# maelaubert/VulkanSift

Hardware: AMD Instinct MI355X
Metric: SIFT detect+match frames/sec (640x480, ~2k kp) (higher is better)
Workload: dtype f32

## Files before the change

### include/vksift_hip.h

```cpp
#ifndef VKSIFT_HIP_H
#define VKSIFT_HIP_H

#include <stddef.h>
#include <stdint.h>

#ifdef __cplusplus
extern "C"
{
#endif

#define VKSIFT_HIP_MAX_TAPS 20
#define VKSIFT_HIP_MATCH_CHUNKS 32
#define VKSIFT_HIP_MATCH_SMALL_NA 1536u
#define VKSIFT_HIP_MATCH_SMALL_NB 4096u
#define VKSIFT_HIP_MATCH_SCRATCH_U32(na, nb) (2u * (size_t)(na) + (size_t)(nb) + 72u + (size_t)(na) * 16u * VKSIFT_HIP_MATCH_CHUNKS)
#define VKSIFT_HIP_ABI_VERSION 6u
#define VKSIFT_HIP_GATHER_SLOTS 512u
#define VKSIFT_HIP_MATCH_SLOTS 256u
#define VKSIFT_HIP_MATCH_PK_NB 32768u
#define VKSIFT_HIP_MAX_ORI 18
#define VKSIFT_HIP_MAX_OCTAVE_SIDE 16383u

  typedef void *vksift_hip_stream;
  typedef void *vksift_hip_graph;
  typedef void *vksift_hip_event;

  int vksift_hip_init(void);
  uint32_t vksift_hip_abi_version(void);
  int vksift_hip_device_count(void);
  int vksift_hip_device_name(int idx, char *out256);
  int vksift_hip_set_device(int idx);
  size_t vksift_hip_device_free_mem(void);
  void *vksift_hip_malloc(size_t bytes);
  void vksift_hip_free(void *p);
  void *vksift_hip_host_malloc(size_t bytes);
  void vksift_hip_host_free(void *p);
  int vksift_hip_host_register(void *p, size_t bytes);
  int vksift_hip_host_unregister(void *p);
  int vksift_hip_is_pinned(const void *p);
  vksift_hip_stream vksift_hip_stream_create(void);
  void vksift_hip_stream_destroy(vksift_hip_stream s);
  int vksift_hip_stream_sync(vksift_hip_stream s);
  int vksift_hip_stream_busy(vksift_hip_stream s);
  vksift_hip_event vksift_hip_event_create(void);
  void vksift_hip_event_destroy(vksift_hip_event e);
  int vksift_hip_event_record(vksift_hip_event e, vksift_hip_stream s);
  int vksift_hip_event_sync(vksift_hip_event e);
  int vksift_hip_event_busy(vksift_hip_event e);
  float vksift_hip_event_elapsed_ms(vksift_hip_event a, vksift_hip_event b);
  int vksift_hip_stream_wait_event(vksift_hip_stream s, vksift_hip_event e);
  int vksift_hip_capture_begin(vksift_hip_stream s);
  int vksift_hip_capture_end(vksift_hip_stream s, vksift_hip_graph *out);
  int vksift_hip_graph_launch(vksift_hip_graph g, vksift_hip_stream s);
  void vksift_hip_graph_destroy(vksift_hip_graph g);
  int vksift_hip_memcpy_h2d(void *dst, const void *src, size_t n, vksift_hip_stream s);
  int vksift_hip_memcpy_d2h(void *dst, const void *src, size_t n, vksift_hip_stream s);
  int vksift_hip_memcpy_d2d(void *dst, const void *src, size_t n, vksift_hip_stream s);
  int vksift_hip_memcpy2d_d2h(void *dst, size_t dpitch, const void *src, size_t spitch, size_t width_bytes, size_t height, vksift_hip_stream s);
  int vksift_hip_post_words(uint32_t *host_mapped_dst, const uint32_t *src, size_t n_words, vksift_hip_stream s);
  int vksift_hip_memset(void *dst, int value, size_t n, vksift_hip_stream s);
  const char *vksift_hip_error_string(int err);
  void vksift_hip_range_push(const char *name);
  void vksift_hip_range_pop(void);

  enum
  {
    VKSIFT_TUNE_WG_TARGET = 0,
    VKSIFT_TUNE_WIDE_MASK = 1,
    VKSIFT_TUNE_MULTI_MAX = 2,
    VKSIFT_TUNE_REFINE_PTR = 3,
    VKSIFT_TUNE_SCAN_FORM = 4,
    VKSIFT_TUNE_PAIR_FORM = 5,
    VKSIFT_TUNE_PYR_GATE = 6,
    VKSIFT_TUNE_DENSE_ROWS = 7,
    VKSIFT_TUNE_SEED_WG = 8,
    VKSIFT_TUNE_SCAN_BAND = 9,
    VKSIFT_TUNE_TAIL_MULTI = 10,
    VKSIFT_TUNE_ZERO_COPY = 11,
    VKSIFT_TUNE_MIN_MARCH = 12,
    VKSIFT_TUNE_COUNT = 16
  };
  int vksift_hip_tune(int knob, int value);
  int vksift_hip_tune_get(int knob);


  typedef struct
  {
    float *base;
    uint32_t w, h;
    uint32_t pitch;
    uint64_t img_stride;
    uint32_t fp16;
    uint32_t reverse;
  } vksift_hip_Plane;

  int vksift_hip_input_blit(const uint8_t *src, uint32_t sw, uint32_t sh, uint64_t src_img_stride, vksift_hip_Plane dst, uint32_t batch,
                            vksift_hip_stream s);

  int vksift_hip_blur(vksift_hip_Plane src, vksift_hip_Plane dst, const float *taps, uint32_t ntaps, uint32_t batch, vksift_hip_stream s);

  int vksift_hip_blur_pair(vksift_hip_Plane src, vksift_hip_Plane dst1, vksift_hip_Plane dst2, const float *taps1, uint32_t ntaps1, const float *taps2,
                           uint32_t ntaps2, uint32_t batch, vksift_hip_stream s);

  int vksift_hip_blur_form(vksift_hip_Plane src, vksift_hip_Plane dst, uint32_t ntaps, uint32_t batch);

  int vksift_hip_blur_multi(const vksift_hip_Plane *src, const vksift_hip_Plane *dst, uint32_t n, const float *taps, uint32_t ntaps, uint32_t batch,
                            vksift_hip_stream s);

  int vksift_hip_blur_downsample(vksift_hip_Plane src, vksift_hip_Plane dst, vksift_hip_Plane next, const float *taps, uint32_t ntaps, uint32_t batch,
                                 vksift_hip_stream s);

  int vksift_hip_seed_upsampled(const uint8_t *src, uint32_t sw, uint32_t sh, uint64_t src_img_stride, vksift_hip_Plane dst, const float *taps, uint32_t ntaps,
                                uint32_t batch, vksift_hip_stream s);

  int vksift_hip_seed_direct(const uint8_t *src, uint32_t sw, uint32_t sh, uint64_t src_img_stride, vksift_hip_Plane dst, const float *taps, uint32_t ntaps,
                             uint32_t batch, vksift_hip_stream s);

  int vksift_hip_downsample(vksift_hip_Plane src, vksift_hip_Plane dst, uint32_t batch, vksift_hip_stream s);

  int vksift_hip_octave_chain(const vksift_hip_Plane *layers, uint32_t n_oct, uint32_t n_layers, uint32_t S, const float *taps, const uint32_t *ntaps,
                              uint32_t batch, vksift_hip_stream s);

  int vksift_hip_dog_plane(const float *lo, const float *hi, uint32_t w, uint32_t h, uint32_t pitch, uint32_t fp16, float *out_dense, vksift_hip_stream s);

  typedef struct
  {
    float *gauss;
    uint32_t fp16;
    uint32_t w, h, pitch;
    uint64_t plane_stride;
    uint64_t img_stride;
    uint32_t S;
    int32_t octave_idx;
    float seed_sigma;
    float dog_threshold;
    float edge_limit;
    uint8_t *feats;
    uint64_t feat_img_stride;
    uint32_t cap;
    uint32_t *found;
    uint32_t found_img_stride;
    uint64_t *seg_mask;
    uint32_t *seg_off;
    uint64_t seg_img_stride;
    uint32_t *cand_xy;
    uint32_t *cand_flag;
    uint32_t *cand_n;
    uint64_t cand_img_stride;
    uint32_t cand_cap;
    float *ori_ang;
    uint32_t *ori_cnt;
    uint64_t ori_img_stride;
    uint32_t max_ori;
    uint32_t use_vlfeat;
    const float *desc_fp_tab;
    uint32_t desc_fp_tab_len;
    uint32_t scan_reverse;
    uint32_t masks_cleared;
    uint32_t sec_index;
  } vksift_hip_OctaveJob;

  typedef struct
  {
    uint8_t *desc;
    uint64_t desc_img_stride;
    uint32_t *norm;
    uint64_t norm_img_stride;
    uint32_t *n;
    uint32_t n_img_stride;
    uint32_t nsec;
    uint32_t sec_cap[16];
    uint8_t *post;
    uint64_t post_img_stride;
    uint32_t *found_post;
    uint32_t found_post_n;
  } vksift_hip_DenseRows;

  int vksift_hip_extract_keypoints(const vksift_hip_OctaveJob *job, uint32_t batch, vksift_hip_stream s, vksift_hip_event scan_done);
  int vksift_hip_orientations(const vksift_hip_OctaveJob *job, uint32_t batch, vksift_hip_stream s);
  int vksift_hip_descriptors(const vksift_hip_OctaveJob *job, uint32_t batch, vksift_hip_stream s);
  int vksift_hip_extract_keypoints_multi(const vksift_hip_OctaveJob *jobs, uint32_t n_jobs, uint32_t batch, vksift_hip_stream s, vksift_hip_event scan_done);
  int vksift_hip_clear_segment_masks(const vksift_hip_OctaveJob *jobs, uint32_t n_jobs, uint32_t batch, vksift_hip_stream s);
  int vksift_hip_selftest_inrange(uint32_t n, uint32_t seed, uint32_t *d_mismatches, vksift_hip_stream s);
  int vksift_hip_orientations_multi(const vksift_hip_OctaveJob *jobs, uint32_t n_jobs, uint32_t batch, vksift_hip_stream s);
  int vksift_hip_descriptors_multi(const vksift_hip_OctaveJob *jobs, uint32_t n_jobs, uint32_t batch, vksift_hip_stream s);
  int vksift_hip_descriptors_multi_dense(const vksift_hip_OctaveJob *jobs, uint32_t n_jobs, uint32_t batch, const vksift_hip_DenseRows *dense,
                                         vksift_hip_stream s);

  int vksift_hip_gather_descriptors(const uint8_t *feats, uint32_t n, uint8_t *desc, vksift_hip_stream s);
  size_t vksift_hip_match_scratch_u32(uint32_t na, uint32_t nb);
  int vksift_hip_match_2nn_desc(const uint8_t *desc_a, uint32_t na, uint32_t a_index_base, const uint8_t *desc_b, uint32_t nb, uint32_t *norm_scratch,
                                size_t scratch_u32, uint8_t *matches, vksift_hip_stream s);
  int vksift_hip_shifted_norms(const uint8_t *desc, uint32_t n, uint32_t *norms, vksift_hip_stream s);
  int vksift_hip_match_2nn_prenormed(const uint8_t *desc_a, const uint32_t *norm_a, uint32_t na, uint32_t a_index_base, const uint8_t *desc_b,
                                     const uint32_t *norm_b, uint32_t nb, uint32_t *scratch, size_t scratch_u32, uint8_t *matches, vksift_hip_stream s);

  int vksift_hip_filter_matches(const uint8_t *fwd, uint64_t fwd_slot_stride, const uint8_t *rev, uint64_t rev_slot_stride, const uint32_t *n_fwd,
                                uint32_t n_stride, float ratio, uint32_t nslots, uint8_t *out, uint64_t out_slot_stride, uint32_t *out_n, vksift_hip_stream s);

  int vksift_hip_pack_features(const uint8_t *feats_base, uint64_t buf_stride, const uint32_t *buf_ids, const uint32_t *out_rows, uint32_t nslots, uint32_t nsec,
                               const uint32_t *sec_off, const uint32_t *sec_cap, const uint32_t *found_base, uint32_t found_buf_stride, uint8_t *out,
                               uint32_t max_rows, uint32_t *found_post, vksift_hip_stream s);
  int vksift_hip_gather_sections(const uint8_t *feats_base, uint64_t buf_stride, const uint32_t *buf_ids, uint32_t nslots, uint32_t nsec,
                                 const uint32_t *sec_off, const uint32_t *sec_cap, const uint32_t *fixed_counts, const uint32_t *found_base,
                                 uint32_t found_buf_stride, uint32_t max_rows, uint32_t pad_rows_to, uint8_t *desc, uint64_t desc_stride,
                                 uint32_t *norms, uint64_t norm_stride, uint32_t *n_out_dev, uint32_t n_stride, vksift_hip_stream s);
  int vksift_hip_match_2nn_async(const uint8_t *cache_desc, const uint32_t *cache_norm, const uint32_t *cache_n, const uint32_t *ids_a, const uint32_t *ids_b,
                                 uint32_t max_na, uint32_t max_nb, uint32_t nb_exact, uint32_t *redo, uint32_t *n_dev, uint8_t *matches, uint32_t nslots, uint64_t cache_desc_stride,
                                 uint64_t cache_norm_stride, uint64_t redo_slot_stride, uint64_t match_slot_stride, uint32_t n_slot_stride,
                                 uint32_t *partial_scratch, vksift_hip_stream s);

  int vksift_hip_gather_correspondences(const uint8_t *feats_base, uint64_t buf_stride, const uint32_t *found_base, uint32_t found_buf_stride,
                                        const uint32_t *slot_tab, const uint32_t *layouts, const uint8_t *filtered, uint64_t filtered_slot_stride,
                                        const uint32_t *filtered_n, uint32_t max_n, uint32_t nslots, float *corr, uint64_t corr_slot_stride, vksift_hip_stream s);
  size_t vksift_hip_ransac_scratch_u32(uint32_t nslots, uint32_t nb_hypotheses);
  int vksift_hip_ransac_homography(const float *corr, uint64_t corr_slot_stride, const uint32_t *n_dev, uint32_t n_stride, uint32_t max_n, uint32_t nslots,
                                   uint32_t nb_hypotheses, float threshold_px, uint64_t seed, uint8_t *results, uint8_t *masks, uint64_t mask_slot_stride,
                                   uint32_t *scratch, size_t scratch_u32, vksift_hip_stream s);
  int vksift_hip_ransac_fundamental(const float *corr, uint64_t corr_slot_stride, const uint32_t *n_dev, uint32_t n_stride, uint32_t max_n, uint32_t nslots,
                                    uint32_t nb_hypotheses, float threshold_px, uint64_t seed, uint8_t *results, uint8_t *masks, uint64_t mask_slot_stride,
                                    uint32_t *scratch, size_t scratch_u32, vksift_hip_stream s);

#define VKSIFT_HIP_GUIDE_HOMOGRAPHY 0u
#define VKSIFT_HIP_GUIDE_FUNDAMENTAL 1u
  int vksift_hip_gather_xy(const uint8_t *feats_base, uint64_t buf_stride, const uint32_t *found_base, uint32_t found_buf_stride, const uint32_t *slot_tab,
                           const uint32_t *layouts, uint32_t max_n, uint32_t nslots, float *xy, uint64_t xy_side_stride, vksift_hip_stream s);
  size_t vksift_hip_guided_scratch_u32(uint32_t nslots, uint32_t max_n);
  int vksift_hip_match_guided(const uint8_t *cache_desc, uint64_t cache_desc_stride, const uint32_t *cache_norm, uint64_t cache_norm_stride, const uint32_t *slot_tab,
                              uint32_t slot_tab_stride, const float *xy, uint64_t xy_side_stride, const uint32_t *n_dev, uint32_t n_stride, uint32_t max_n,
                              const float *models, uint32_t model_stride, const uint32_t *valid, uint32_t valid_stride, uint32_t model_kind, float t2, float ratio,
                              float max_distance, uint32_t cross_check, uint32_t nslots, uint8_t *out, uint64_t out_slot_stride, uint32_t *out_n, uint32_t *scratch,
                              size_t scratch_u32, vksift_hip_stream s);

#ifdef __cplusplus
}
#endif
#endif
```

### vulkansift_amd/csrc/hip/extrema.hip

```cpp
#include <hip/hip_runtime.h>
#include <type_traits>
#include <stdint.h>
#include <stdlib.h>

#include "../detmath.h"
#include "multi.h"
#include "vksift_hip.h"

namespace
{

struct DogView
{
  const float *base;
  int w, h, pitch;
  size_t plane;
  int S;
  int fp16;
};

template <bool F16>
__device__ __forceinline__ float ld(const DogView &d, int s, int x, int y)
{
  if (s < 0 || s > d.S + 1)
    return 0.f;
  if (F16)
  {
    const _Float16 *p = (const _Float16 *)d.base + (size_t)s * d.plane + (size_t)y * d.pitch + x;
    return (float)(_Float16)((float)p[d.plane] - (float)p[0]);
  }
  const float *p = d.base + (size_t)s * d.plane + (size_t)y * d.pitch + x;
  return p[d.plane] - p[0];
}

struct KpRecord
{
  float x, y, scale_x, scale_y;
  uint32_t scale_idx;
  int32_t octave_idx;
  float sigma, orientation, intensity;
};

template <bool F16>
__device__ bool refine_texel(const DogView &d, int x, int y, int s, float dog_threshold, float edge_limit, float seed_sigma, int octave_idx, KpRecord *kp)
{
  const int W = d.w, H = d.h, S = d.S;
  float oX = 0.f, oY = 0.f, oS = 0.f, gX = 0.f, gY = 0.f, gS = 0.f;
  int rx = x, ry = y, rs = s;
  for (int step = 0; step < 5; step++)
  {
    float vc = ld<F16>(d, rs, rx, ry);
    float sp = ld<F16>(d, rs + 1, rx, ry), sm = ld<F16>(d, rs - 1, rx, ry);
    float xp = ld<F16>(d, rs, rx + 1, ry), xm = ld<F16>(d, rs, rx - 1, ry);
    float yp = ld<F16>(d, rs, rx, ry + 1), ym = ld<F16>(d, rs, rx, ry - 1);
    gS = 0.5f * (sp - sm);
    gX = 0.5f * (xp - xm);
    gY = 0.5f * (yp - ym);
    float h11 = sp + sm - 2.f * vc;
    float h22 = xp + xm - 2.f * vc;
    float h33 = yp + ym - 2.f * vc;
    float h12 = 0.25f * (ld<F16>(d, rs + 1, rx + 1, ry) - ld<F16>(d, rs + 1, rx - 1, ry) - ld<F16>(d, rs - 1, rx + 1, ry) + ld<F16>(d, rs - 1, rx - 1, ry));
    float h13 = 0.25f * (ld<F16>(d, rs + 1, rx, ry + 1) - ld<F16>(d, rs + 1, rx, ry - 1) - ld<F16>(d, rs - 1, rx, ry + 1) + ld<F16>(d, rs - 1, rx, ry - 1));
    float h23 = 0.25f * (ld<F16>(d, rs, rx + 1, ry + 1) - ld<F16>(d, rs, rx + 1, ry - 1) - ld<F16>(d, rs, rx - 1, ry + 1) + ld<F16>(d, rs, rx - 1, ry - 1));

    float det = h11 * ((h22 * h33) - (h23 * h23)) - h12 * ((h12 * h33) - (h13 * h23)) + h13 * ((h12 * h23) - (h13 * h22));
    if (det == 0.0f)
      return false;
    float i11 = ((h22 * h33) - (h23 * h23)) / det;
    float i12 = -1.f * ((h12 * h33) - (h13 * h23)) / det;
    float i13 = ((h12 * h23) - (h13 * h22)) / det;
    float i22 = ((h11 * h33) - (h13 * h13)) / det;
    float i23 = -1.f * ((h11 * h23) - (h13 * h12)) / det;
    float i33 = ((h11 * h22) - (h12 * h12)) / det;
    oS = -i11 * gS - i12 * gX - i13 * gY;
    oX = -i12 * gS - i22 * gX - i23 * gY;
    oY = -i13 * gS - i23 * gX - i33 * gY;

    if (fabsf(oX) < 0.6f && fabsf(oY) < 0.6f && fabsf(oS) < 0.6f)
      break;
    else if (step < 4)
    {
      rx += ((oX >= 0.6f && rx < (W - 2)) ? 1 : 0) + ((oX <= -0.6f && rx > 1) ? -1 : 0);
      ry += ((oY >= 0.6f && ry < (H - 2)) ? 1 : 0) + ((oY <= -0.6f && ry > 1) ? -1 : 0);
      rs += ((oS >= 0.6f && rs < (S + 1)) ? 1 : 0) + ((oS <= -0.6f && rs > 1) ? -1 : 0);
    }
  }
  float sx = (float)rx + oX, sy = (float)ry + oY, ss = (float)rs + oS;
  float vc = ld<F16>(d, rs, rx, ry);
  float nv = vc + 0.5f * (gX * oX + gY * oY + gS * oS);
  if (!(fabsf(nv) > dog_threshold && fabsf(oX) < 1.5f && fabsf(oY) < 1.5f && fabsf(oS) < 1.5f && sx >= 0 && sx < (float)W && sy >= 0 && sy < (float)H &&
        ss >= 0 && ss <= (float)(S + 1)))
    return false;
  float e11 = ld<F16>(d, rs, rx + 1, ry) + ld<F16>(d, rs, rx - 1, ry) - 2.f * vc;
  float e22 = ld<F16>(d, rs, rx, ry + 1) + ld<F16>(d, rs, rx, ry - 1) - 2.f * vc;
  float e12 = 0.25f * (ld<F16>(d, rs, rx + 1, ry + 1) - ld<F16>(d, rs, rx + 1, ry - 1) - ld<F16>(d, rs, rx - 1, ry + 1) + ld<F16>(d, rs, rx - 1, ry - 1));
  float edgeness = ((e11 + e22) * (e11 + e22)) / ((e11 * e22) - (e12 * e12));
  if (!((edgeness < edge_limit) && (edgeness >= 0)))
    return false;

  float scale_factor = octave_idx >= 0 ? dm_pow2i(octave_idx) : 1.f / dm_pow2i(-octave_idx);
  kp->scale_x = sx;
  kp->scale_y = sy;
  kp->scale_idx = (uint32_t)roundf(ss);
  kp->octave_idx = octave_idx;
  kp->sigma = seed_sigma * dm_exp2f(ss / (float)S) * scale_factor;
  kp->orientation = 0.f;
  kp->intensity = nv;
  kp->x = sx * scale_factor;
  kp->y = sy * scale_factor;
  return true;
}

template <bool F16>
__device__ bool refine_texel_buf(const __amdgpu_buffer_rsrc_t rsrc, int W, int H, int pitch, unsigned plane, int S, int x, int y, int s, float dog_threshold,
                                 float edge_limit, float seed_sigma, int octave_idx, KpRecord *kp)
{
  constexpr unsigned EB = F16 ? 2u : 4u;
  const int pitch_b = pitch * (int)EB;
  const unsigned plane_b = plane * EB;
  auto tex = [&](unsigned base, int row_off) -> float {
    if (F16)
      return (float)__builtin_bit_cast(_Float16, (unsigned short)__builtin_amdgcn_raw_buffer_load_b16(rsrc, base, row_off, 0));
    return __uint_as_float(__builtin_amdgcn_raw_buffer_load_b32(rsrc, base, row_off, 0));
  };
  auto dog = [&](float hi, float lo) -> float { return F16 ? (float)(_Float16)(hi - lo) : hi - lo; };
  float oX = 0.f, oY = 0.f, oS = 0.f, gX = 0.f, gY = 0.f, gS = 0.f;
  float vc = 0.f, xp = 0.f, xm = 0.f, yp = 0.f, ym = 0.f, h23 = 0.f;
  int rx = x, ry = y, rs = s;
  for (int step = 0; step < 5; step++)
  {
    const unsigned b0 = ((unsigned)rs * plane + (unsigned)(ry - 1) * (unsigned)pitch + (unsigned)(rx - 1)) * EB;
    const unsigned bm = b0 - plane_b, b1 = b0 + plane_b, b2 = b1 + plane_b;
    float g0[3][3], g1[3][3];
#pragma unroll
    for (int j = 0; j < 3; j++)
#pragma unroll
      for (int i = 0; i < 3; i++)
      {
        g0[j][i] = tex(b0 + (unsigned)i * EB, j * pitch_b);
        g1[j][i] = tex(b1 + (unsigned)i * EB, j * pitch_b);
      }
    const float gm_c = tex(bm + EB, pitch_b), gm_xm = tex(bm, pitch_b), gm_xp = tex(bm + 2u * EB, pitch_b), gm_ym = tex(bm + EB, 0), gm_yp = tex(bm + EB, 2 * pitch_b);
    const float g2_c = tex(b2 + EB, pitch_b), g2_xm = tex(b2, pitch_b), g2_xp = tex(b2 + 2u * EB, pitch_b), g2_ym = tex(b2 + EB, 0), g2_yp = tex(b2 + EB, 2 * pitch_b);
    const bool up = rs + 1 <= S + 1;
    const float sp = up ? dog(g2_c, g1[1][1]) : 0.f, sm = dog(g0[1][1], gm_c);
    const float p_xp = up ? dog(g2_xp, g1[1][2]) : 0.f, p_xm = up ? dog(g2_xm, g1[1][0]) : 0.f;
    const float p_yp = up ? dog(g2_yp, g1[2][1]) : 0.f, p_ym = up ? dog(g2_ym, g1[0][1]) : 0.f;
    const float m_xp = dog(g0[1][2], gm_xp), m_xm = dog(g0[1][0], gm_xm), m_yp = dog(g0[2][1], gm_yp), m_ym = dog(g0[0][1], gm_ym);
    float d0[3][3];
#pragma unroll
    for (int j = 0; j < 3; j++)
#pragma unroll
      for (int i = 0; i < 3; i++)
        d0[j][i] = dog(g1[j][i], g0[j][i]);
    vc = d0[1][1];
    xp = d0[1][2], xm = d0[1][0], yp = d0[2][1], ym = d0[0][1];
    gS = 0.5f * (sp - sm);
    gX = 0.5f * (xp - xm);
    gY = 0.5f * (yp - ym);
    float h11 = sp + sm - 2.f * vc;
    float h22 = xp + xm - 2.f * vc;
    float h33 = yp + ym - 2.f * vc;
    float h12 = 0.25f * (p_xp - p_xm - m_xp + m_xm);
    float h13 = 0.25f * (p_yp - p_ym - m_yp + m_ym);
    h23 = 0.25f * (d0[2][2] - d0[0][2] - d0[2][0] + d0[0][0]);

    float det = h11 * ((h22 * h33) - (h23 * h23)) - h12 * ((h12 * h33) - (h13 * h23)) + h13 * ((h12 * h23) - (h13 * h22));
    if (det == 0.0f)
      return false;
    float i11 = ((h22 * h33) - (h23 * h23)) / det;
    float i12 = -1.f * ((h12 * h33) - (h13 * h23)) / det;
    float i13 = ((h12 * h23) - (h13 * h22)) / det;
    float i22 = ((h11 * h33) - (h13 * h13)) / det;
    float i23 = -1.f * ((h11 * h23) - (h13 * h12)) / det;
    float i33 = ((h11 * h22) - (h12 * h12)) / det;
    oS = -i11 * gS - i12 * gX - i13 * gY;
    oX = -i12 * gS - i22 * gX - i23 * gY;
    oY = -i13 * gS - i23 * gX - i33 * gY;

    if (fabsf(oX) < 0.6f && fabsf(oY) < 0.6f && fabsf(oS) < 0.6f)
      break;
    else if (step < 4)
    {
      rx += ((oX >= 0.6f && rx < (W - 2)) ? 1 : 0) + ((oX <= -0.6f && rx > 1) ? -1 : 0);
      ry += ((oY >= 0.6f && ry < (H - 2)) ? 1 : 0) + ((oY <= -0.6f && ry > 1) ? -1 : 0);
      rs += ((oS >= 0.6f && rs < (S + 1)) ? 1 : 0) + ((oS <= -0.6f && rs > 1) ? -1 : 0);
    }
  }
  float sx = (float)rx + oX, sy = (float)ry + oY, ss = (float)rs + oS;
  float nv = vc + 0.5f * (gX * oX + gY * oY + gS * oS);
  if (!(fabsf(nv) > dog_threshold && fabsf(oX) < 1.5f && fabsf(oY) < 1.5f && fabsf(oS) < 1.5f && sx >= 0 && sx < (float)W && sy >= 0 && sy < (float)H &&
        ss >= 0 && ss <= (float)(S + 1)))
    return false;
  float e11 = xp + xm - 2.f * vc;
  float e22 = yp + ym - 2.f * vc;
  float e12 = h23;
  float edgeness = ((e11 + e22) * (e11 + e22)) / ((e11 * e22) - (e12 * e12));
  if (!((edgeness < edge_limit) && (edgeness >= 0)))
    return false;

  float scale_factor = octave_idx >= 0 ? dm_pow2i(octave_idx) : 1.f / dm_pow2i(-octave_idx);
  kp->scale_x = sx;
  kp->scale_y = sy;
  kp->scale_idx = (uint32_t)roundf(ss);
  kp->octave_idx = octave_idx;
  kp->sigma = seed_sigma * dm_exp2f(ss / (float)S) * scale_factor;
  kp->orientation = 0.f;
  kp->intensity = nv;
  kp->x = sx * scale_factor;
  kp->y = sy * scale_factor;
  return true;
}

struct ExtremaArgs
{
  const float *gauss;
  int fp16;
  int w, h, pitch;
  uint64_t plane_stride, img_stride;
  int S, octave_idx;
  float seed_sigma, dog_threshold, edge_limit;
  uint64_t *seg_mask;
  uint32_t *seg_off;
  uint64_t seg_img_stride;
  int nseg;
  uint8_t *feats;
  uint64_t feat_img_stride;
  uint32_t cap;
  uint32_t *found;
  uint32_t found_img_stride;
  uint32_t *cand_xy;
  uint32_t *cand_flag;
  uint32_t *cand_n;
  uint64_t cand_img_stride;
  uint32_t cand_cap;
  int band;
  uint32_t nsegs;
  uint32_t nchunks;
  int scan_rev;
};

__device__ __forceinline__ float wave_shr1(float v, float edge)
{
  return __builtin_bit_cast(float, __builtin_amdgcn_update_dpp(__builtin_bit_cast(int, edge), __builtin_bit_cast(int, v), 0x138, 0xf, 0xf, false));
}
__device__ __forceinline__ float wave_shl1(float v, float edge)
{
  return __builtin_bit_cast(float, __builtin_amdgcn_update_dpp(__builtin_bit_cast(int, edge), __builtin_bit_cast(int, v), 0x130, 0xf, 0xf, false));
}

__device__ __forceinline__ float fmax2(float a, float b)
{
  float r;
  asm("v_max_f32 %0, %1, %2" : "=v"(r) : "v"(a), "v"(b));
  return r;
}
__device__ __forceinline__ float fmin2(float a, float b)
{
  float r;
  asm("v_min_f32 %0, %1, %2" : "=v"(r) : "v"(a), "v"(b));
  return r;
}
__device__ __forceinline__ float fmax3(float a, float b, float c)
{
  float r;
  asm("v_max3_f32 %0, %1, %2, %3" : "=v"(r) : "v"(a), "v"(b), "v"(c));
  return r;
}
__device__ __forceinline__ float fmin3(float a, float b, float c)
{
  float r;
  asm("v_min3_f32 %0, %1, %2, %3" : "=v"(r) : "v"(a), "v"(b), "v"(c));
  return r;
}

__device__ __forceinline__ unsigned long long spread32(unsigned long long x)
{
  x &= 0xFFFFFFFFull;
  x = (x | (x << 16)) & 0x0000FFFF0000FFFFull;
  x = (x | (x << 8)) & 0x00FF00FF00FF00FFull;
  x = (x | (x << 4)) & 0x0F0F0F0F0F0F0F0Full;
  x = (x | (x << 2)) & 0x3333333333333333ull;
  x = (x | (x << 1)) & 0x5555555555555555ull;
  return x;
}

typedef unsigned u32x2_t __attribute__((ext_vector_type(2)));
constexpr unsigned EXT_OOB = 0x80000000u;

template <int S, int NSLOT, bool F16>
__global__ void __launch_bounds__(256, 4) k_extrema_lean(Multi<ExtremaArgs> m, int strip_major)
{
  const VBlock vb = vblock(m);
  const ExtremaArgs &a = m.oct[vb.o];
  const int band = a.band;
  constexpr int NL = S + 2;
  constexpr int EB = F16 ? 2 : 4;
  constexpr int AHEAD = NSLOT - 3;
  const int lane = threadIdx.x & 63;
  const int wv = __builtin_amdgcn_readfirstlane((int)(threadIdx.x >> 6));
  int b = vb.z;
  int bx = vb.x, by = vb.y * 4 + wv;
  if (strip_major)
  {
    unsigned blk = vb.y * vb.gx + vb.x;
    if (strip_major & 2)
    {
      const unsigned per_img = vb.gx * vb.gy, total = per_img * vb.gz;
      if ((total & 7u) == 0)
      {
        const unsigned n = blk + per_img * vb.z, per = total >> 3, k = n >> 3;
        const unsigned wi = (n & 7u) * per + (a.scan_rev ? per - 1u - k : k);
        b = (int)(wi / per_img);
        blk = wi - (unsigned)b * per_img;
      }
    }
    const unsigned id = blk * 4u + (unsigned)wv, ns = (unsigned)(a.nseg + 1) / 2u;
    by = (int)(id / ns), bx = (int)(id - (unsigned)by * ns);
  }
  const int y0 = by * band;
  if (y0 >= a.h)
    return;
  const int y1 = min(y0 + band, a.h);
  const int x0 = bx * 128, x = x0 + 2 * lane;
  const uint8_t *img = (const uint8_t *)a.gauss + (size_t)b * a.img_stride * EB;
  const int pitch4 = a.pitch * EB;
  __amdgpu_buffer_rsrc_t rs[NL + 1];
#pragma unroll
  for (int l = 0; l <= NL; l++)
    rs[l] = __builtin_amdgcn_make_buffer_rsrc((void *)(img + (size_t)l * a.plane_stride * EB), 0, a.pitch * a.h * EB, 0x00020000);
  const unsigned off2 = x < a.pitch ? (unsigned)x * (unsigned)EB : EXT_OOB;
  const int hx = lane == 0 ? x0 - 1 : x0 + 128;
  const unsigned offh = ((lane == 0 || lane == 63) && hx >= 0 && hx < a.pitch) ? (unsigned)hx * (unsigned)EB : EXT_OOB;
  const unsigned long long colA = __ballot(x >= 1 && x < a.w - 1), colB = __ballot(x + 1 < a.w - 1);
  const float pre = a.dog_threshold * 0.8f;
  const int seg0 = bx * 2;
  const bool has_seg1 = seg0 + 1 < a.nseg;
  const int ylo = max(y0, 1), yhi = min(y1, a.h - 1);
  const bool odd = lane & 1;
  const unsigned half = (unsigned)lane >> 1;

  u32x2_t wv2[NSLOT][NL + 1];
  unsigned wh[NSLOT][NL + 1];
  auto fetch_row = [&](int r, auto SLOT) {
    constexpr int slot = decltype(SLOT)::value;
    const int rr = min(max(r, 0), a.h - 1);
    const int so = rr * pitch4;
#pragma unroll
    for (int l = 0; l <= NL; l++)
    {
      if (F16)
      {
        wv2[slot][l].x = __builtin_amdgcn_raw_buffer_load_b32(rs[l], off2, so, 0);
        wh[slot][l] = (unsigned)__builtin_amdgcn_raw_buffer_load_b16(rs[l], offh, so, 0);
      }
      else
      {
        wv2[slot][l] = __builtin_amdgcn_raw_buffer_load_b64(rs[l], off2, so, 0);
        wh[slot][l] = __builtin_amdgcn_raw_buffer_load_b32(rs[l], offh, so, 0);
      }
    }
  };
  typedef _Float16 h2x __attribute__((ext_vector_type(2)));
  auto to_dog = [&](auto SLOT) {
    constexpr int slot = decltype(SLOT)::value;
    if (F16)
    {
      float lo0, lo1, loh;
      {
        const h2x t = __builtin_bit_cast(h2x, wv2[slot][0].x);
        lo0 = (float)t.x, lo1 = (float)t.y;
        loh = (float)__builtin_bit_cast(h2x, wh[slot][0]).x;
      }
#pragma unroll
      for (int l = 0; l < NL; l++)
      {
        const h2x t = __builtin_bit_cast(h2x, wv2[slot][l + 1].x);
        const float hi0 = (float)t.x, hi1 = (float)t.y, hih = (float)__builtin_bit_cast(h2x, wh[slot][l + 1]).x;
        wv2[slot][l].x = __float_as_uint((float)(_Float16)(hi0 - lo0));
        wv2[slot][l].y = __float_as_uint((float)(_Float16)(hi1 - lo1));
        wh[slot][l] = __float_as_uint((float)(_Float16)(hih - loh));
        lo0 = hi0, lo1 = hi1, loh = hih;
      }
      return;
    }
#pragma unroll
    for (int l = 0; l < NL; l++)
    {
      wv2[slot][l].x = __float_as_uint(__uint_as_float(wv2[slot][l + 1].x) - __uint_as_float(wv2[slot][l].x));
      wv2[slot][l].y = __float_as_uint(__uint_as_float(wv2[slot][l + 1].y) - __uint_as_float(wv2[slot][l].y));
      wh[slot][l] = __float_as_uint(__uint_as_float(wh[slot][l + 1]) - __uint_as_float(wh[slot][l]));
    }
  };

  auto phase = [&](auto PC, int r) {
    constexpr int P = decltype(PC)::value;
    constexpr int sn = P, sm = (P + NSLOT - 1) % NSLOT, so_ = (P + NSLOT - 2) % NSLOT, sf = (P + AHEAD) % NSLOT;
    if (r + AHEAD <= y1)
      fetch_row(r + AHEAD, std::integral_constant<int, sf>{});
    to_dog(std::integral_constant<int, sn>{});
    const int y = r - 1;
    if (y < ylo || y >= yhi)
      return;
    float ownxA[S], ownnA[S], ownxB[S], ownnB[S], fullxA[NL], fullnA[NL], fullxB[NL], fullnB[NL];
#pragma unroll
    for (int l = 0; l < NL; l++)
    {
      const float ao = __uint_as_float(wv2[so_][l].x), am = __uint_as_float(wv2[sm][l].x), an = __uint_as_float(wv2[sn][l].x);
      const float bo = __uint_as_float(wv2[so_][l].y), bm = __uint_as_float(wv2[sm][l].y), bn = __uint_as_float(wv2[sn][l].y);
      const float ho = __uint_as_float(wh[so_][l]), hm = __uint_as_float(wh[sm][l]), hn = __uint_as_float(wh[sn][l]);
      const float vxa = fmax3(ao, am, an), vna = fmin3(ao, am, an);
      const float vxb = fmax3(bo, bm, bn), vnb = fmin3(bo, bm, bn);
      const float vxh = fmax3(ho, hm, hn), vnh = fmin3(ho, hm, hn);
      const float Lx = wave_shr1(vxb, vxh), Ln = wave_shr1(vnb, vnh);
      const float Rx = wave_shl1(vxa, vxh), Rn = wave_shl1(vna, vnh);
      if (l >= 1 && l <= S)
      {
        ownxA[l - 1] = fmax3(Lx, vxb, fmax2(ao, an)), ownnA[l - 1] = fmin3(Ln, vnb, fmin2(ao, an));
        ownxB[l - 1] = fmax3(vxa, Rx, fmax2(bo, bn)), ownnB[l - 1] = fmin3(vna, Rn, fmin2(bo, bn));
      }
      fullxA[l] = fmax3(Lx, vxa, vxb), fullnA[l] = fmin3(Ln, vna, vnb);
      fullxB[l] = fmax3(vxa, vxb, Rx), fullnB[l] = fmin3(vna, vnb, Rn);
    }
#pragma unroll
    for (int sz = 0; sz < S; sz++)
    {
      const int l = sz + 1;
      const float ca = __uint_as_float(wv2[sm][l].x), cb = __uint_as_float(wv2[sm][l].y);
      const float nxa = fmax3(ownxA[sz], fullxA[l - 1], fullxA[l + 1]), nna = fmin3(ownnA[sz], fullnA[l - 1], fullnA[l + 1]);
      const float nxb = fmax3(ownxB[sz], fullxB[l - 1], fullxB[l + 1]), nnb = fmin3(ownnB[sz], fullnB[l - 1], fullnB[l + 1]);
      const unsigned long long ma = (__ballot(ca > nxa) | __ballot(ca < nna)) & __ballot(fabsf(ca) > pre) & colA;
      const unsigned long long mb = (__ballot(cb > nxb) | __ballot(cb < nnb)) & __ballot(fabsf(cb) > pre) & colB;
      if ((ma | mb) != 0ull)
      {
        const unsigned lo = odd ? (unsigned)mb : (unsigned)ma, hi = odd ? (unsigned)(mb >> 32) : (unsigned)(ma >> 32);
        const unsigned long long m0 = __ballot((lo >> half) & 1u), m1 = __ballot((hi >> half) & 1u);
        if (lane == 0)
        {
          const size_t base = ((size_t)sz * a.h + y) * a.nseg + (size_t)b * a.seg_img_stride;
          a.seg_mask[base + seg0] = m0;
          if (has_seg1)
            a.seg_mask[base + seg0 + 1] = m1;
        }
      }
    }
  };

  if (AHEAD >= 1)
    fetch_row(y0 - 1, std::integral_constant<int, 0>{});
  if (AHEAD >= 2)
    fetch_row(y0, std::integral_constant<int, 1 % NSLOT>{});
  int r = y0 - 1;
  for (;;)
  {
    phase(std::integral_constant<int, 0>{}, r);
    if (++r > y1)
      break;
    phase(std::integral_constant<int, 1>{}, r);
    if (++r > y1)
      break;
    phase(std::integral_constant<int, 2>{}, r);
    if (++r > y1)
      break;
    phase(std::integral_constant<int, 3>{}, r);
    if (++r > y1)
      break;
    if (NSLOT > 4)
    {
      phase(std::integral_constant<int, 4 % NSLOT>{}, r);
      if (++r > y1)
        break;
    }
  }
}

constexpr uint32_t SEG_CHUNK = 4096;

__global__ void __launch_bounds__(1024) k_segment_scan(Multi<ExtremaArgs> m)
{
  __shared__ uint32_t wave_tot[16];
  const VBlock vb = vblock(m);
  const ExtremaArgs &a = m.oct[vb.o];
  const int b = (int)vb.y;
  const uint64_t *__restrict__ mask = a.seg_mask + (size_t)b * a.seg_img_stride;
  uint32_t *__restrict__ off = a.seg_off + (size_t)b * a.seg_img_stride;
  uint32_t *__restrict__ chunk_tot = a.cand_flag;
  const uint64_t chunk_img_stride = a.cand_img_stride;
  const uint32_t n = a.nsegs;
  const int lane = threadIdx.x & 63, wave = threadIdx.x >> 6;
  const uint32_t i0 = vb.x * SEG_CHUNK + 4u * threadIdx.x;
  uint32_t p[4];
#pragma unroll
  for (int k = 0; k < 4; k++)
    p[k] = i0 + k < n ? (uint32_t)__popcll(mask[i0 + k]) : 0u;
  const uint32_t tsum = p[0] + p[1] + p[2] + p[3];
  uint32_t incl = tsum;
#pragma unroll
  for (int dlt = 1; dlt < 64; dlt <<= 1)
  {
    uint32_t t = __shfl_up(incl, dlt, 64);
    if (lane >= dlt)
      incl += t;
  }
  if (lane == 63)
    wave_tot[wave] = incl;
  __syncthreads();
  uint32_t wave_base = 0, total = 0;
  for (int wv = 0; wv < 16; wv++)
  {
    if (wv < wave)
      wave_base += wave_tot[wv];
    total += wave_tot[wv];
  }
  uint32_t run = wave_base + incl - tsum;
#pragma unroll
  for (int k = 0; k < 4; k++)
  {
    if (i0 + k < n)
      off[i0 + k] = run;
    run += p[k];
  }
  if (threadIdx.x == 0)
    chunk_tot[(size_t)b * chunk_img_stride + vb.x] = total;
}


__global__ void __launch_bounds__(256) k_cand_list(Multi<ExtremaArgs> mu)
{
  const VBlock vb = vblock(mu);
  const ExtremaArgs &a = mu.oct[vb.o];
  const uint32_t seg = vb.x * 256 + threadIdx.x;
  const int b = (int)vb.y;
  const uint32_t *chunk_tot = a.cand_flag + (size_t)b * a.cand_img_stride;
  if (vb.x == 0 && threadIdx.x == 0)
  {
    uint32_t total = 0;
    for (uint32_t c = 0; c < a.nchunks; c++)
      total += chunk_tot[c];
    a.cand_n[b] = total;
    if (total == 0)
      a.found[(size_t)b * a.found_img_stride] = 0;
  }
  unsigned long long m = seg < a.nsegs ? a.seg_mask[seg + (size_t)b * a.seg_img_stride] : 0ull;
  if (__ballot(m != 0ull) == 0ull)
    return;
  uint32_t base = 0;
  for (uint32_t c = threadIdx.x & 63u, nc = (vb.x * 256u) / SEG_CHUNK; c < nc; c += 64u)
    base += chunk_tot[c];
#pragma unroll
  for (int dlt = 32; dlt >= 1; dlt >>= 1)
    base += __shfl_xor(base, dlt, 64);
  if (m == 0ull)
    return;
  uint32_t pos = a.seg_off[seg + (size_t)b * a.seg_img_stride] + base;
  const uint32_t segx = seg % (uint32_t)a.nseg;
  const uint32_t yy = (seg / (uint32_t)a.nseg) % (uint32_t)a.h;
  const uint32_t sz = seg / ((uint32_t)a.nseg * (uint32_t)a.h);
  uint32_t *out = a.cand_xy + (size_t)b * a.cand_img_stride;
  while (m)
  {
    const int bit = __ffsll((long long)m) - 1;
    m &= m - 1;
    if (pos < a.cand_cap)
      out[pos] = (segx * 64u + (uint32_t)bit) | (yy << 14) | ((sz + 1u) << 28);
    pos++;
  }
}

template <bool F16, bool BUF>
__global__ void __launch_bounds__(256) k_refine_flags(Multi<ExtremaArgs> m)
{
  __shared__ uint32_t s_cnt[4];
  const VBlock vb = vblock(m);
  const ExtremaArgs &a = m.oct[vb.o];
  const int b = (int)vb.x;
  uint32_t n = a.cand_n[b];
  n = n < a.cand_cap ? n : a.cand_cap;
  const uint32_t nch = (n + 255u) / 256u;
  DogView d{(const float *)((const uint8_t *)a.gauss + (size_t)b * a.img_stride * (a.fp16 ? 2u : 4u)), a.w, a.h, a.pitch, (size_t)a.plane_stride, a.S, a.fp16};
  const __amdgpu_buffer_rsrc_t rsrc =
      __builtin_amdgcn_make_buffer_rsrc((void *)d.base, 0, (int)((unsigned)(a.S + 3) * (unsigned)a.plane_stride * (F16 ? 2u : 4u)), 0x00020000);
  const uint32_t *xy = a.cand_xy + (size_t)b * a.cand_img_stride;
  uint32_t *flag = a.cand_flag + (size_t)b * a.cand_img_stride;
  uint32_t *chunk_sum = a.seg_off + (size_t)b * a.seg_img_stride;
  for (uint32_t chunk = vb.y; chunk < nch; chunk += vb.gy)
  {
    const uint32_t i = chunk * 256u + threadIdx.x;
    bool ok = false;
    if (i < n)
    {
      const uint32_t c = xy[i];
      KpRecord kp;
      const int cx = (int)(c & 0x3fffu), cy = (int)((c >> 14) & 0x3fffu), cs = (int)(c >> 28);
      ok = BUF ? refine_texel_buf<F16>(rsrc, a.w, a.h, a.pitch, (unsigned)a.plane_stride, a.S, cx, cy, cs, a.dog_threshold, a.edge_limit, a.seed_sigma, a.octave_idx, &kp)
               : refine_texel<F16>(d, cx, cy, cs, a.dog_threshold, a.edge_limit, a.seed_sigma, a.octave_idx, &kp);
      flag[i] = ok ? 1u : 0u;
    }
    const unsigned long long bal = __ballot(ok);
    if ((threadIdx.x & 63) == 0)
      s_cnt[threadIdx.x >> 6] = (uint32_t)__popcll(bal);
    __syncthreads();
    if (threadIdx.x == 0)
      chunk_sum[chunk] = s_cnt[0] + s_cnt[1] + s_cnt[2] + s_cnt[3];
    __syncthreads();
  }
}

template <bool F16, bool BUF>
__global__ void __launch_bounds__(256) k_cand_emit(Multi<ExtremaArgs> m)
{
  __shared__ uint32_t s_cnt[4];
  __shared__ uint32_t s_red[4];
  __shared__ uint32_t s_list[256];
  const VBlock vb = vblock(m);
  const ExtremaArgs &a = m.oct[vb.o];
  const int b = (int)vb.x;
  const int lane = threadIdx.x & 63, wave = threadIdx.x >> 6;
  uint32_t n = a.cand_n[b];
  n = n < a.cand_cap ? n : a.cand_cap;
  const uint32_t nch = (n + 255u) / 256u;
  DogView d{(const float *)((const uint8_t *)a.gauss + (size_t)b * a.img_stride * (a.fp16 ? 2u : 4u)), a.w, a.h, a.pitch, (size_t)a.plane_stride, a.S, a.fp16};
  const __amdgpu_buffer_rsrc_t rsrc =
      __builtin_amdgcn_make_buffer_rsrc((void *)d.base, 0, (int)((unsigned)(a.S + 3) * (unsigned)a.plane_stride * (F16 ? 2u : 4u)), 0x00020000);
  const uint32_t *xy = a.cand_xy + (size_t)b * a.cand_img_stride;
  const uint32_t *flag = a.cand_flag + (size_t)b * a.cand_img_stride;
  const uint32_t *chunk_sum = a.seg_off + (size_t)b * a.seg_img_stride;
  for (uint32_t chunk = vb.y; chunk < nch; chunk += vb.gy)
  {
    uint32_t part = 0;
    for (uint32_t c = threadIdx.x; c < chunk; c += 256u)
      part += chunk_sum[c];
#pragma unroll
    for (int dlt = 32; dlt >= 1; dlt >>= 1)
      part += __shfl_xor(part, dlt, 64);
    const uint32_t i = chunk * 256u + threadIdx.x;
    const bool v = i < n && flag[i] != 0u;
    const unsigned long long bal = __ballot(v);
    if (lane == 0)
      s_cnt[wave] = (uint32_t)__popcll(bal), s_red[wave] = part;
    __syncthreads();
    const uint32_t cbase = s_red[0] + s_red[1] + s_red[2] + s_red[3];
    uint32_t rank = (uint32_t)__popcll(bal & ((1ull << lane) - 1ull));
    for (int wv = 0; wv < wave; wv++)
      rank += s_cnt[wv];
    const uint32_t total = s_cnt[0] + s_cnt[1] + s_cnt[2] + s_cnt[3];
    if (v)
      s_list[rank] = xy[i];
    __syncthreads();
    const uint32_t idx = cbase + threadIdx.x;
    if (chunk + 1u == nch && threadIdx.x == 0)
      a.found[(size_t)b * a.found_img_stride] = cbase + total;
    if (threadIdx.x < total && idx < a.cap)
    {
      const uint32_t c = s_list[threadIdx.x];
      KpRecord kp;
      const int cx = (int)(c & 0x3fffu), cy = (int)((c >> 14) & 0x3fffu), cs = (int)(c >> 28);
      if (BUF)
        refine_texel_buf<F16>(rsrc, a.w, a.h, a.pitch, (unsigned)a.plane_stride, a.S, cx, cy, cs, a.dog_threshold, a.edge_limit, a.seed_sigma, a.octave_idx, &kp);
      else
        refine_texel<F16>(d, cx, cy, cs, a.dog_threshold, a.edge_limit, a.seed_sigma, a.octave_idx, &kp);
      uint32_t *rec = (uint32_t *)(a.feats + (size_t)b * a.feat_img_stride + (size_t)idx * 164);
      rec[0] = __float_as_uint(kp.x);
      rec[1] = __float_as_uint(kp.y);
      rec[2] = __float_as_uint(kp.scale_x);
      rec[3] = __float_as_uint(kp.scale_y);
      rec[4] = kp.scale_idx;
      rec[5] = (uint32_t)kp.octave_idx;
      rec[6] = __float_as_uint(kp.sigma);
      rec[7] = __float_as_uint(kp.orientation);
      rec[8] = __float_as_uint(kp.intensity);
    }
    __syncthreads();
  }
}

}

static int make_extrema_args(const vksift_hip_OctaveJob *job, ExtremaArgs *out)
{
  if (job->w == 0u || job->h == 0u || job->w > VKSIFT_HIP_MAX_OCTAVE_SIDE || job->h > VKSIFT_HIP_MAX_OCTAVE_SIDE || job->S == 0u || job->S > 13u)
    return (int)hipErrorInvalidValue;
  const uint64_t eb = job->fp16 ? 2u : 4u;
  if (job->pitch < job->w || job->plane_stride < (uint64_t)job->pitch * job->h || (uint64_t)job->pitch * job->h * eb >= 0x80000000ull)
    return (int)hipErrorInvalidValue;
  if (((uintptr_t)job->gauss & 3u) != 0u || (job->fp16 && ((job->pitch | job->plane_stride | job->img_stride) & 1u) != 0u))
    return (int)hipErrorInvalidValue;
  ExtremaArgs a;
  a.gauss = job->gauss;
  a.fp16 = (int)job->fp16;
  a.w = (int)job->w, a.h = (int)job->h, a.pitch = (int)job->pitch;
  a.plane_stride = job->plane_stride, a.img_stride = job->img_stride;
  a.S = (int)job->S, a.octave_idx = job->octave_idx;
  a.seed_sigma = job->seed_sigma, a.dog_threshold = job->dog_threshold, a.edge_limit = job->edge_limit;
  a.seg_mask = job->seg_mask, a.seg_off = job->seg_off, a.seg_img_stride = job->seg_img_stride;
  a.nseg = (int)((job->w + 63) / 64);
  a.feats = job->feats, a.feat_img_stride = job->feat_img_stride, a.cap = job->cap;
  a.found = job->found, a.found_img_stride = job->found_img_stride;
  a.cand_xy = job->cand_xy, a.cand_flag = job->cand_flag, a.cand_n = job->cand_n;
  a.cand_img_stride = job->cand_img_stride, a.cand_cap = job->cand_cap;
  a.scan_rev = (int)job->scan_reverse;
  a.band = job->h > 256u ? 48 : 16;
  if (vksift_hip_tune_get(VKSIFT_TUNE_SCAN_BAND) > 0 && job->h > 256u)
    a.band = vksift_hip_tune_get(VKSIFT_TUNE_SCAN_BAND);
  a.nsegs = job->S * job->h * (uint32_t)a.nseg;
  a.nchunks = (a.nsegs + SEG_CHUNK - 1u) / SEG_CHUNK;
  if (job->seg_img_stride != a.nsegs || a.nchunks > a.cand_cap || job->cand_img_stride < job->cand_cap)
    return (int)hipErrorInvalidValue;
  *out = a;
  return 0;
}

static int clear_masks(const ExtremaArgs *args, uint32_t n, uint32_t batch, hipStream_t hs)
{
  for (uint32_t i = 0; i < n;)
  {
    uint32_t j = i + 1;
    size_t bytes = sizeof(uint64_t) * (size_t)args[i].nsegs * batch;
    while (j < n && (const uint8_t *)args[j].seg_mask == (const uint8_t *)args[i].seg_mask + bytes)
      bytes += sizeof(uint64_t) * (size_t)args[j].nsegs * batch, j++;
    const hipError_t me = hipMemsetAsync(args[i].seg_mask, 0, bytes, hs);
    if (me != hipSuccess)
      return (int)me;
    i = j;
  }
  return 0;
}

static int extract_run(const vksift_hip_OctaveJob *jobs, uint32_t n, uint32_t batch, hipStream_t hs, hipEvent_t scan_done)
{
  ExtremaArgs args[MULTI_MAX];
  for (uint32_t i = 0; i < n; i++)
  {
    const int e = make_extrema_args(&jobs[i], &args[i]);
    if (e)
      return e;
  }
  const bool f16 = args[0].fp16 != 0;
  const int S = args[0].S;
  {
    uint64_t waves = 0;
    for (uint32_t i = 0; i < n; i++)
      waves += (uint64_t)batch * ((args[i].w + 127) / 128) * ((args[i].h + args[i].band - 1) / args[i].band);
    if (waves < 2048u && vksift_hip_tune_get(VKSIFT_TUNE_SCAN_BAND) <= 0)
      for (uint32_t i = 0; i < n; i++)
        args[i].band = 16;
  }

  bool cleared = true;
  for (uint32_t i = 0; i < n; i++)
    cleared = cleared && jobs[i].masks_cleared != 0;
  if (!cleared)
  {
    const int me = clear_masks(args, n, batch, hs);
    if (me)
      return me;
  }
  const int sm = 3;
  for (uint32_t i = 0; i < n; i++)
    if ((uint64_t)jobs[i].pitch * jobs[i].h * (f16 ? 2u : 4u) >= 0x80000000ull)
      return (int)hipErrorInvalidValue;

#define VKSIFT_MULTI(M, GX, GY, GZ)                              \
  Multi<ExtremaArgs> M;                                           \
  M.n = 0;                                                        \
  for (uint32_t i = 0; i < n; i++)                                \
  {                                                               \
    const ExtremaArgs &a = args[i];                               \
    (void)a;                                                      \
    if (!multi_add(M, args[i], (GX), (GY), (GZ)))                 \
      return (int)hipErrorInvalidValue;                           \
  }
  {
    VKSIFT_MULTI(ms, (uint32_t)(a.nseg + 1) / 2u, ((a.h + a.band - 1) / a.band + 3u) / 4u, batch)
    const dim3 sgrid(ms.start[ms.n]);
    switch (S)
    {
#define VKSIFT_CASE(N)                                                                \
  case N:                                                                             \
    if (f16)                                                                          \
      hipLaunchKernelGGL((k_extrema_lean<N, 5, true>), sgrid, dim3(256), 0, hs, ms, sm);  \
    else                                                                              \
      hipLaunchKernelGGL((k_extrema_lean<N, 4, false>), sgrid, dim3(256), 0, hs, ms, sm); \
    break;
      VKSIFT_CASE(1) VKSIFT_CASE(2) VKSIFT_CASE(3) VKSIFT_CASE(4) VKSIFT_CASE(5) VKSIFT_CASE(6) VKSIFT_CASE(7) VKSIFT_CASE(8) VKSIFT_CASE(9)
      VKSIFT_CASE(10) VKSIFT_CASE(11) VKSIFT_CASE(12) VKSIFT_CASE(13)
#undef VKSIFT_CASE
    default:
      return (int)hipErrorInvalidValue;
    }
  }
  if (scan_done)
    (void)hipEventRecord(scan_done, hs);
  {
    VKSIFT_MULTI(m2, a.nchunks, batch, 1u)
    hipLaunchKernelGGL(k_segment_scan, dim3(m2.start[m2.n]), dim3(1024), 0, hs, m2);
  }
  {
    VKSIFT_MULTI(m3, (a.nsegs + 255u) / 256u, batch, 1u)
    hipLaunchKernelGGL(k_cand_list, dim3(m3.start[m3.n]), dim3(256), 0, hs, m3);
  }
  const uint32_t rcap = 65536u / batch < 16u ? 16u : (65536u / batch > 512u ? 512u : 65536u / batch);
#define VKSIFT_REFINE_CHUNKS(a) (((uint64_t)(a).S * (uint32_t)(a).w * (uint32_t)(a).h / 4u + 64u + 255u) / 256u)
  VKSIFT_MULTI(mr, batch, VKSIFT_REFINE_CHUNKS(a) > rcap ? rcap : (uint32_t)VKSIFT_REFINE_CHUNKS(a), 1u)
#undef VKSIFT_REFINE_CHUNKS
  const dim3 rgrid(mr.start[mr.n]);
  bool buf = vksift_hip_tune_get(VKSIFT_TUNE_REFINE_PTR) == 0;
  for (uint32_t i = 0; i < n; i++)
    buf = buf && (uint64_t)(args[i].S + 3) * args[i].plane_stride * (f16 ? 2u : 4u) < 0x7FFF0000ull;
  if (f16 && buf)
    hipLaunchKernelGGL((k_refine_flags<true, true>), rgrid, dim3(256), 0, hs, mr);
  else if (f16)
    hipLaunchKernelGGL((k_refine_flags<true, false>), rgrid, dim3(256), 0, hs, mr);
  else if (buf)
    hipLaunchKernelGGL((k_refine_flags<false, true>), rgrid, dim3(256), 0, hs, mr);
  else
    hipLaunchKernelGGL((k_refine_flags<false, false>), rgrid, dim3(256), 0, hs, mr);
  if (f16 && buf)
    hipLaunchKernelGGL((k_cand_emit<true, true>), rgrid, dim3(256), 0, hs, mr);
  else if (f16)
    hipLaunchKernelGGL((k_cand_emit<true, false>), rgrid, dim3(256), 0, hs, mr);
  else if (buf)
    hipLaunchKernelGGL((k_cand_emit<false, true>), rgrid, dim3(256), 0, hs, mr);
  else
    hipLaunchKernelGGL((k_cand_emit<false, false>), rgrid, dim3(256), 0, hs, mr);
#undef VKSIFT_MULTI
  return (int)hipGetLastError();
}

extern "C" int vksift_hip_extract_keypoints_multi(const vksift_hip_OctaveJob *jobs, uint32_t n_jobs, uint32_t batch, vksift_hip_stream s,
                                                  vksift_hip_event scan_done)
{
  if (n_jobs == 0 || batch == 0)
    return 0;
  for (uint32_t i = 0; i < n_jobs; i++)
  {
    ExtremaArgs a;
    const int e = make_extrema_args(&jobs[i], &a);
    if (e)
      return e;
  }
  for (uint32_t i0 = 0; i0 < n_jobs;)
  {
    uint32_t i1 = i0 + 1;
    while (i1 < n_jobs && i1 - i0 < multi_run_max() && jobs[i1].S == jobs[i0].S && jobs[i1].fp16 == jobs[i0].fp16)
      i1++;
    const int e = extract_run(jobs + i0, i1 - i0, batch, (hipStream_t)s, i1 == n_jobs ? (hipEvent_t)scan_done : nullptr);
    if (e)
      return e;
    i0 = i1;
  }
  return 0;
}

extern "C" int vksift_hip_clear_segment_masks(const vksift_hip_OctaveJob *jobs, uint32_t n_jobs, uint32_t batch, vksift_hip_stream s)
{
  if (n_jobs == 0 || batch == 0)
    return 0;
  if (n_jobs > 16)
    return (int)hipErrorInvalidValue;
  ExtremaArgs args[16];
  for (uint32_t i = 0; i < n_jobs; i++)
  {
    const int e = make_extrema_args(&jobs[i], &args[i]);
    if (e)
      return e;
  }
  return clear_masks(args, n_jobs, batch, (hipStream_t)s);
}

extern "C" int vksift_hip_extract_keypoints(const vksift_hip_OctaveJob *job, uint32_t batch, vksift_hip_stream s, vksift_hip_event scan_done)
{
  return vksift_hip_extract_keypoints_multi(job, 1, batch, s, scan_done);
}
```

Before: 25150.

## Compact nonempty segment list in scan so candidate listing launches per chunk

The segment scan now packs a nonempty-segment count alongside candidate counts and writes a compact per-chunk list of nonempty segments with their offsets. Candidate listing launches one block per 4096-segment chunk and walks only that list, instead of one thread per segment across the whole image. Refine and emit blocks now exit early when they have no chunk, and emit keeps a running prefix sum across grid-stride iterations rather than recomputing it. A tune knob lets the refine grid cap be overridden. The cost is more bit-packing logic and limits on chunk size enforced by static asserts.

```diff
diff --git a/include/vksift_hip.h b/include/vksift_hip.h
--- a/include/vksift_hip.h
+++ b/include/vksift_hip.h
@@ -78,6 +78,7 @@
     VKSIFT_TUNE_TAIL_MULTI = 10,
     VKSIFT_TUNE_ZERO_COPY = 11,
     VKSIFT_TUNE_MIN_MARCH = 12,
+    VKSIFT_TUNE_REFINE_GRID = 13,
     VKSIFT_TUNE_COUNT = 16
   };
   int vksift_hip_tune(int knob, int value);
diff --git a/vulkansift_amd/csrc/hip/extrema.hip b/vulkansift_amd/csrc/hip/extrema.hip
--- a/vulkansift_amd/csrc/hip/extrema.hip
+++ b/vulkansift_amd/csrc/hip/extrema.hip
@@ -475,25 +475,37 @@
 }
 
 constexpr uint32_t SEG_CHUNK = 4096;
-
-__global__ void __launch_bounds__(1024) k_segment_scan(Multi<ExtremaArgs> m)
-{
-  __shared__ uint32_t wave_tot[16];
+constexpr uint32_t SEG_NE_SHIFT = 19;
+constexpr uint32_t SEG_CAND_MASK = (1u << SEG_NE_SHIFT) - 1u;
+constexpr uint32_t SEG_ENTRY_SHIFT = 12;
+static_assert(SEG_CHUNK * 64u < (1u << SEG_NE_SHIFT) && SEG_CHUNK < (1u << (32 - SEG_NE_SHIFT)), "the packed scan word holds a chunk's sums");
+static_assert(SEG_CHUNK == (1u << SEG_ENTRY_SHIFT) && SEG_CHUNK * 64u <= (1u << (32 - SEG_ENTRY_SHIFT)), "a list entry holds segment and offset");
+
+constexpr uint32_t SCAN_THREADS = 1024;
+constexpr uint32_t SCAN_PER = SEG_CHUNK / SCAN_THREADS;
+constexpr uint32_t SCAN_WAVES = SCAN_THREADS / 64;
+
+__global__ void __launch_bounds__(SCAN_THREADS) k_segment_scan(Multi<ExtremaArgs> m)
+{
+  __shared__ uint32_t wave_tot[SCAN_WAVES];
   const VBlock vb = vblock(m);
   const ExtremaArgs &a = m.oct[vb.o];
   const int b = (int)vb.y;
   const uint64_t *__restrict__ mask = a.seg_mask + (size_t)b * a.seg_img_stride;
-  uint32_t *__restrict__ off = a.seg_off + (size_t)b * a.seg_img_stride;
+  uint32_t *__restrict__ list = a.seg_off + (size_t)b * a.seg_img_stride + (size_t)vb.x * SEG_CHUNK;
   uint32_t *__restrict__ chunk_tot = a.cand_flag;
   const uint64_t chunk_img_stride = a.cand_img_stride;
   const uint32_t n = a.nsegs;
   const int lane = threadIdx.x & 63, wave = threadIdx.x >> 6;
-  const uint32_t i0 = vb.x * SEG_CHUNK + 4u * threadIdx.x;
-  uint32_t p[4];
-#pragma unroll
-  for (int k = 0; k < 4; k++)
-    p[k] = i0 + k < n ? (uint32_t)__popcll(mask[i0 + k]) : 0u;
-  const uint32_t tsum = p[0] + p[1] + p[2] + p[3];
+  const uint32_t l0 = SCAN_PER * threadIdx.x, i0 = vb.x * SEG_CHUNK + l0;
+  uint32_t p[SCAN_PER], tsum = 0;
+#pragma unroll
+  for (uint32_t k = 0; k < SCAN_PER; k++)
+  {
+    const uint32_t c = i0 + k < n ? (uint32_t)__popcll(mask[i0 + k]) : 0u;
+    p[k] = c | (c != 0u ? 1u << SEG_NE_SHIFT : 0u);
+    tsum += p[k];
+  }
   uint32_t incl = tsum;
 #pragma unroll
   for (int dlt = 1; dlt < 64; dlt <<= 1)
@@ -506,7 +518,7 @@
     wave_tot[wave] = incl;
   __syncthreads();
   uint32_t wave_base = 0, total = 0;
-  for (int wv = 0; wv < 16; wv++)
+  for (int wv = 0; wv < (int)SCAN_WAVES; wv++)
   {
     if (wv < wave)
       wave_base += wave_tot[wv];
@@ -514,10 +526,10 @@
   }
   uint32_t run = wave_base + incl - tsum;
 #pragma unroll
-  for (int k = 0; k < 4; k++)
-  {
-    if (i0 + k < n)
-      off[i0 + k] = run;
+  for (uint32_t k = 0; k < SCAN_PER; k++)
+  {
+    if (p[k] != 0u)
+      list[run >> SEG_NE_SHIFT] = (l0 + k) | ((run & SEG_CAND_MASK) << SEG_ENTRY_SHIFT);
     run += p[k];
   }
   if (threadIdx.x == 0)
@@ -529,41 +541,46 @@
 {
   const VBlock vb = vblock(mu);
   const ExtremaArgs &a = mu.oct[vb.o];
-  const uint32_t seg = vb.x * 256 + threadIdx.x;
   const int b = (int)vb.y;
   const uint32_t *chunk_tot = a.cand_flag + (size_t)b * a.cand_img_stride;
   if (vb.x == 0 && threadIdx.x == 0)
   {
     uint32_t total = 0;
     for (uint32_t c = 0; c < a.nchunks; c++)
-      total += chunk_tot[c];
+      total += chunk_tot[c] & SEG_CAND_MASK;
     a.cand_n[b] = total;
     if (total == 0)
       a.found[(size_t)b * a.found_img_stride] = 0;
   }
-  unsigned long long m = seg < a.nsegs ? a.seg_mask[seg + (size_t)b * a.seg_img_stride] : 0ull;
-  if (__ballot(m != 0ull) == 0ull)
+  const uint32_t nent = chunk_tot[vb.x] >> SEG_NE_SHIFT;
+  if (nent == 0u)
     return;
   uint32_t base = 0;
-  for (uint32_t c = threadIdx.x & 63u, nc = (vb.x * 256u) / SEG_CHUNK; c < nc; c += 64u)
-    base += chunk_tot[c];
+  for (uint32_t c = threadIdx.x & 63u; c < vb.x; c += 64u)
+    base += chunk_tot[c] & SEG_CAND_MASK;
 #pragma unroll
   for (int dlt = 32; dlt >= 1; dlt >>= 1)
     base += __shfl_xor(base, dlt, 64);
-  if (m == 0ull)
-    return;
-  uint32_t pos = a.seg_off[seg + (size_t)b * a.seg_img_stride] + base;
-  const uint32_t segx = seg % (uint32_t)a.nseg;
-  const uint32_t yy = (seg / (uint32_t)a.nseg) % (uint32_t)a.h;
-  const uint32_t sz = seg / ((uint32_t)a.nseg * (uint32_t)a.h);
+  const uint32_t *list = a.seg_off + (size_t)b * a.seg_img_stride + (size_t)vb.x * SEG_CHUNK;
+  const uint64_t *mask = a.seg_mask + (size_t)b * a.seg_img_stride;
   uint32_t *out = a.cand_xy + (size_t)b * a.cand_img_stride;
-  while (m)
-  {
-    const int bit = __ffsll((long long)m) - 1;
-    m &= m - 1;
-    if (pos < a.cand_cap)
-      out[pos] = (segx * 64u + (uint32_t)bit) | (yy << 14) | ((sz + 1u) << 28);
-    pos++;
+  for (uint32_t j = threadIdx.x; j < nent; j += 256u)
+  {
+    const uint32_t e = list[j];
+    const uint32_t seg = vb.x * SEG_CHUNK + (e & (SEG_CHUNK - 1u));
+    uint32_t pos = base + (e >> SEG_ENTRY_SHIFT);
+    unsigned long long m = mask[seg];
+    const uint32_t segx = seg % (uint32_t)a.nseg;
+    const uint32_t yy = (seg / (uint32_t)a.nseg) % (uint32_t)a.h;
+    const uint32_t sz = seg / ((uint32_t)a.nseg * (uint32_t)a.h);
+    while (m)
+    {
+      const int bit = __ffsll((long long)m) - 1;
+      m &= m - 1;
+      if (pos < a.cand_cap)
+        out[pos] = (segx * 64u + (uint32_t)bit) | (yy << 14) | ((sz + 1u) << 28);
+      pos++;
+    }
   }
 }
 
@@ -577,6 +594,8 @@
   uint32_t n = a.cand_n[b];
   n = n < a.cand_cap ? n : a.cand_cap;
   const uint32_t nch = (n + 255u) / 256u;
+  if (vb.y >= nch)
+    return;
   DogView d{(const float *)((const uint8_t *)a.gauss + (size_t)b * a.img_stride * (a.fp16 ? 2u : 4u)), a.w, a.h, a.pitch, (size_t)a.plane_stride, a.S, a.fp16};
   const __amdgpu_buffer_rsrc_t rsrc =
       __builtin_amdgcn_make_buffer_rsrc((void *)d.base, 0, (int)((unsigned)(a.S + 3) * (unsigned)a.plane_stride * (F16 ? 2u : 4u)), 0x00020000);
@@ -619,17 +638,21 @@
   uint32_t n = a.cand_n[b];
   n = n < a.cand_cap ? n : a.cand_cap;
   const uint32_t nch = (n + 255u) / 256u;
+  if (vb.y >= nch)
+    return;
   DogView d{(const float *)((const uint8_t *)a.gauss + (size_t)b * a.img_stride * (a.fp16 ? 2u : 4u)), a.w, a.h, a.pitch, (size_t)a.plane_stride, a.S, a.fp16};
   const __amdgpu_buffer_rsrc_t rsrc =
       __builtin_amdgcn_make_buffer_rsrc((void *)d.base, 0, (int)((unsigned)(a.S + 3) * (unsigned)a.plane_stride * (F16 ? 2u : 4u)), 0x00020000);
   const uint32_t *xy = a.cand_xy + (size_t)b * a.cand_img_stride;
   const uint32_t *flag = a.cand_flag + (size_t)b * a.cand_img_stride;
   const uint32_t *chunk_sum = a.seg_off + (size_t)b * a.seg_img_stride;
+  uint32_t share = 0, summed = 0;
   for (uint32_t chunk = vb.y; chunk < nch; chunk += vb.gy)
   {
-    uint32_t part = 0;
-    for (uint32_t c = threadIdx.x; c < chunk; c += 256u)
-      part += chunk_sum[c];
+    for (uint32_t c = summed + threadIdx.x; c < chunk; c += 256u)
+      share += chunk_sum[c];
+    summed = chunk;
+    uint32_t part = share;
 #pragma unroll
     for (int dlt = 32; dlt >= 1; dlt >>= 1)
       part += __shfl_xor(part, dlt, 64);
@@ -793,13 +816,12 @@
     (void)hipEventRecord(scan_done, hs);
   {
     VKSIFT_MULTI(m2, a.nchunks, batch, 1u)
-    hipLaunchKernelGGL(k_segment_scan, dim3(m2.start[m2.n]), dim3(1024), 0, hs, m2);
-  }
-  {
-    VKSIFT_MULTI(m3, (a.nsegs + 255u) / 256u, batch, 1u)
-    hipLaunchKernelGGL(k_cand_list, dim3(m3.start[m3.n]), dim3(256), 0, hs, m3);
-  }
-  const uint32_t rcap = 65536u / batch < 16u ? 16u : (65536u / batch > 512u ? 512u : 65536u / batch);
+    hipLaunchKernelGGL(k_segment_scan, dim3(m2.start[m2.n]), dim3(SCAN_THREADS), 0, hs, m2);
+    hipLaunchKernelGGL(k_cand_list, dim3(m2.start[m2.n]), dim3(256), 0, hs, m2);
+  }
+  uint32_t rcap = 65536u / batch < 16u ? 16u : (65536u / batch > 512u ? 512u : 65536u / batch);
+  if (vksift_hip_tune_get(VKSIFT_TUNE_REFINE_GRID) > 0)
+    rcap = (uint32_t)vksift_hip_tune_get(VKSIFT_TUNE_REFINE_GRID);
 #define VKSIFT_REFINE_CHUNKS(a) (((uint64_t)(a).S * (uint32_t)(a).w * (uint32_t)(a).h / 4u + 64u + 255u) / 256u)
   VKSIFT_MULTI(mr, batch, VKSIFT_REFINE_CHUNKS(a) > rcap ? rcap : (uint32_t)VKSIFT_REFINE_CHUNKS(a), 1u)
 #undef VKSIFT_REFINE_CHUNKS
```

After: 25380, median of 6. No clear change (+0.9%).
